# wbhart/mpir-fft

Measured on AMD Instinct MI355X. Metric: limbs/s for new_mpn_mul N×N-bit at 1/2/4/8 MI355X; % HBM roofline, higher is better.
Workload: dtype u64; 1 GPU; C3: new_mpn_mul depth=15 w=4 n1=n2=20312500 limbs (l=2048 limbs/coeff, NC x NR = 256 x 256, trunc=39936); parallelism=single

## Files before the change

### __graft_entry__.py

```python
import os
import subprocess
import sys

ROOT = os.path.dirname(os.path.abspath(__file__))
CSRC = os.path.join(ROOT, "mpir-fft_amd", "csrc")
LIB = os.path.join(ROOT, "mpir-fft_amd", "libmpfft.so")
HIPCC = os.environ.get("HIPCC", "/opt/rocm/bin/hipcc")


def build_lib(force=False):
    if force:
        subprocess.run(["make", "-s", "-C", CSRC, "clean"], check=True)
    jobs = str(min(8, os.cpu_count() or 1))
    subprocess.run(["make", "-s", "-C", CSRC, "-j" + jobs, "HIPCC=" + HIPCC], check=True)
    subprocess.run(["make", "-s", "-C", CSRC, "-j" + jobs, "HIPCC=" + HIPCC, "pwspill"], check=True)


def build_oracle():
    subprocess.run(["make", "-s", "-C", os.path.join(ROOT, "oracle")], check=True)


def build_c_caller():
    subprocess.run(["make", "-s", "-C", os.path.join(ROOT, "tests", "c_abi")], check=True)
    subprocess.run(["make", "-s", "-C", os.path.join(ROOT, "tests", "c_sqr")], check=True)


def build_host_tests():
    subprocess.run(["make", "-s", "-C", os.path.join(ROOT, "tests", "pw_host")], check=True)
    subprocess.run(["make", "-s", "-C", os.path.join(ROOT, "tests", "split_prune_host")], check=True)
    subprocess.run(["make", "-s", "-C", os.path.join(ROOT, "tests", "pw_sqr_host")], check=True)


def build():
    build_lib()
    build_oracle()
    build_c_caller()
    build_host_tests()
    sys.path.insert(0, ROOT)
    import mpfft_loader
    m = mpfft_loader.load()
    assert m.lib().mpfft_version() >= 1


def smoke():
    import numpy as np
    import torch
    sys.path.insert(0, ROOT)
    sys.path.insert(0, os.path.join(ROOT, "oracle"))
    import mpfft_loader
    import oracle as O
    m = mpfft_loader.load()
    assert torch.cuda.is_available(), "smoke() needs a GPU"
    depth, w, n1, n2 = 9, 2, 120, 97
    a = m.fill_random(n1, 0x1001)
    b = m.fill_random(n2, 0x2002)
    dev = torch.device("cuda:0")
    da = torch.from_numpy(a.view(np.int64)).to(dev)
    db = torch.from_numpy(b.view(np.int64)).to(dev)
    dr = torch.zeros(n1 + n2, dtype=torch.int64, device=dev)
    ws = m.alloc_workspace(n1, n2, depth, w, dev)
    m.mul_device(dr, da, n1, db, n2, depth, w, ws)
    torch.cuda.synchronize()
    got = dr.cpu().numpy().view(np.uint64)
    want = O.new_mpn_mul(a, b, depth, w)
    assert (got == want).all(), "GPU new_mpn_mul differs from the oracle"
    assert O.to_int(got) == O.to_int(a) * O.to_int(b), "GPU product is not the exact product"
    r = np.zeros(n1 + n2, dtype=np.uint64)
    m.new_mpn_mul(r, a, n1, b, n2, depth, w)
    assert (r == want).all()
    d6, w6, m1, m2 = 8, 1, 700, 500
    a6 = m.fill_random(m1, 0x61)
    b6 = m.fill_random(m2, 0x62)
    r6 = m.mul6(a6, b6, d6, w6)
    assert (r6 == O.new_mpn_mul6(a6, b6, d6, w6)).all(), "GPU new_mpn_mul6 differs from the oracle"
    assert O.to_int(r6) == O.to_int(a6) * O.to_int(b6)
    ds = torch.zeros(2 * n1, dtype=torch.int64, device=dev)
    wsq = m.alloc_workspace_sqr(n1, depth, w, dev)
    m.sqr_device(ds, da, n1, depth, w, wsq)
    torch.cuda.synchronize()
    assert O.to_int(ds.cpu().numpy().view(np.uint64)) == O.to_int(a) ** 2, "GPU square is not the exact square"
    print("smoke: ok (depth=%d w=%d n1=%d n2=%d; mul6 depth=%d w=%d n1=%d n2=%d)" % (depth, w, n1, n2, d6, w6, m1, m2))


if __name__ == "__main__":
    build()
    if len(sys.argv) > 1 and sys.argv[1] == "smoke":
        smoke()
```

### mpir-fft_amd/csrc/pkernels.hpp

```cpp
#pragma once
#include <type_traits>
#include "coeff.hpp"

#ifndef PW_TIGHT9
#define PW_TIGHT9 1
#endif
__host__ __device__ constexpr bool pw_tight(int K) { return PW_TIGHT9 && K == 512; }
#ifndef PW_LATE_B_ALL
#define PW_LATE_B_ALL 0
#endif
__host__ __device__ constexpr bool pw_late_b(int K) { return pw_tight(K) || PW_LATE_B_ALL; }
#ifndef PW_LATE_INFL
#define PW_LATE_INFL 1
#endif
#ifndef PW_A_INFL
#define PW_A_INFL 2
#endif
#ifndef PW_QUAD4
#define PW_QUAD4 0
#endif

__host__ __device__ constexpr size_t pw_lds_bytes(int M, int K, int l)
{
    return ((size_t)M * K * 8 > (size_t)l * 4 ? (size_t)M * K * 8 : (size_t)l * 4) + (pw_tight(K) ? 0 : (size_t)K * 8);
}

template <int M, int LK>
__host__ __device__ constexpr int pw_wpe()
{
    return pw_lds_bytes(M, 1 << LK, 64 * M) * (1024 >> LK) <= 160 * 1024 ? 4 : 2;
}
#ifndef PW_PD_TIGHT
#define PW_PD_TIGHT 16
#endif
template <int M, int LK>
#ifndef PW_PD_WIDE
#define PW_PD_WIDE 16
#endif
__host__ __device__ constexpr int pw_pd() { return pw_wpe<M, LK>() == 4 ? (pw_tight(1 << LK) ? PW_PD_TIGHT : PW_PD_WIDE) : 2 * M; }


#ifndef PW_NORM_SPILL_ALL
#define PW_NORM_SPILL_ALL 0
#endif
template <int M>
__host__ __device__ __forceinline__ int pw_norm(u64 (&L)[M], int T)
{
    const int D = T + 1;
#if defined(__HIP_DEVICE_COMPILE__)
    {
        const u32 w0 = (u32)L[0], n0 = w0 - (u32)D;
        const bool spill = PW_NORM_SPILL_ALL || (D > 0 ? w0 < (u32)D : (D < 0 ? n0 < (u32)(-D) : false));
        L[0] = (L[0] & ~0xffffffffull) | (spill ? w0 : n0);
        return spill ? T : -1;
    }
#endif
    const u32 dh = D < 0 ? ~0u : 0u;
    u32 b = 0;
#pragma unroll
    for (int j = 0; j < M; ++j) {
        const u32 lo = __builtin_subc((u32)L[j], j == 0 ? (u32)D : dh, b, &b);
        const u32 hi = __builtin_subc((u32)(L[j] >> 32), dh, b, &b);
        L[j] = ((u64)hi << 32) | lo;
    }
    return (D < 0) - (int)b - 1;
}

template <int M, int LK, int PD = 2 * M, int FIXE = -1>
__host__ __device__ __forceinline__ void pw_combine(u64 (&L)[M], int &T, int &S, int alpha, const u32 *Xw,
                                                   int packed, int q, unsigned E)
{
    constexpr int K = 1 << LK, NW = 2 * M;
    constexpr unsigned NP = 64 * M;
    const int Tq = packed >> 1, Sq = packed & 1;
    bool neg = E >= NP;
    if (neg) E -= NP;
    if (FIXE >= 0) E = (unsigned)FIXE;
    const int Yw = ((int)E - 1) >> 5;
    const unsigned sh = (unsigned)(32 * (Yw + 1)) - E;
    if (alpha == 0) {
#pragma unroll
        for (int j = 0; j < M; ++j) L[j] = 0;
        T = 0;
        S = 0;
    } else if (alpha < 0) {
        S ^= 1;
    }
    neg ^= (S ^ Sq) != 0;
    const u32 smask = neg ? ~0u : 0u;
    const u32 *bn = Xw + q - Yw * K;
    const u32 *bw = bn + NW * K;
    u32 wprev = (-1 < Yw ? bw : bn)[-K] ^ (-1 < Yw ? ~smask : smask);
    u32 c = 1;
    constexpr int D0 = PD < NW ? PD : NW;
    u32 wv[NW];
#pragma unroll
    for (int k = 0; k < D0; ++k) {
        const bool wr = k < Yw;
        wv[k] = (wr ? bw : bn)[k * K];
#if defined(__HIP_DEVICE_COMPILE__)
        if ((k & 7) == 7) __builtin_amdgcn_sched_barrier(0);
#endif
    }
#pragma unroll
    for (int k = 0; k < NW; ++k) {
        if (k + D0 < NW) {
            const bool wr2 = k + D0 < Yw;
            wv[k + D0] = (wr2 ? bw : bn)[(k + D0) * K];
        }
        const bool wr = k < Yw;
        const u32 w = wv[k] ^ (wr ? ~smask : smask);
#if defined(__HIP_DEVICE_COMPILE__)
        const u32 o = __builtin_amdgcn_alignbit(w, wprev, sh);
#else
        const u32 o = (u32)((((u64)w << 32) | wprev) >> sh);
#endif
        wprev = w;
        const u32 lw = (u32)(L[k >> 1] >> (32 * (k & 1)));
        const u32 r = __builtin_addc(lw, o, c, &c);
        if (k & 1) L[k >> 1] = (L[k >> 1] & 0xffffffffull) | ((u64)r << 32);
        else L[k >> 1] = (L[k >> 1] & ~0xffffffffull) | r;
#if defined(__HIP_DEVICE_COMPILE__)
        if (D0 < NW && (k & 3) == 3) __builtin_amdgcn_sched_barrier(0);
#endif
    }
    T += (int)c;
    if (Tq != -1) {
        const int cv = neg ? 1 + Tq : -1 - Tq;
        const i64 d = (i64)cv * ((i64)1 << (32 - sh));
        const u32 dl = (u32)d, dhi = (u32)((u64)d >> 32), sx = d < 0 ? ~0u : 0u;
        u32 cc = 0;
#pragma unroll
        for (int k = 0; k < NW; ++k) {
            const u32 ad = k < Yw ? 0u : k == Yw ? dl : k == Yw + 1 ? dhi : sx;
            const u32 lw = (u32)(L[k >> 1] >> (32 * (k & 1)));
            const u32 r = __builtin_addc(lw, ad, cc, &cc);
            if (k & 1) L[k >> 1] = (L[k >> 1] & 0xffffffffull) | ((u64)r << 32);
            else L[k >> 1] = (L[k >> 1] & ~0xffffffffull) | r;
        }
        T += (int)cc + (Yw == NW - 1 ? (int)(d >> 32) : (d < 0 ? -1 : 0));
    }
}

template <int M>
__host__ __device__ __forceinline__ int pw_canon(u64 (&L)[M], int T)
{
    i128 acc = -(i128)T;
#pragma unroll
    for (int j = 0; j < M; ++j) {
        acc += (i128)L[j];
        L[j] = (u64)acc;
        acc >>= 64;
    }
    const int c1 = (int)(i64)acc;
    acc = -(i128)c1;
#pragma unroll
    for (int j = 0; j < M; ++j) {
        acc += (i128)L[j];
        L[j] = (u64)acc;
        acc >>= 64;
    }
    if ((i64)acc != 0) {
#pragma unroll
        for (int j = 0; j < M; ++j) L[j] = 0;
        return 1;
    }
    return 0;
}

template <int M>
__host__ __device__ __forceinline__ void pw_sqrt2(u64 (&L)[M], int &T)
{
    static_assert(M % 2 == 0, "the half swap needs an even limb count");
    constexpr int H = M / 2;
    i128 a0 = (i128)T, a1 = -(i128)T;
#pragma unroll
    for (int j = 0; j < H; ++j) {
        const u64 lo = L[j], hi = L[j + H];
        a0 += -(i128)hi - (i128)lo;
        a1 += (i128)lo - (i128)hi;
        L[j] = (u64)a0;
        L[j + H] = (u64)a1;
        a0 >>= 64;
        a1 >>= 64;
    }
    i128 c = a0;
#pragma unroll
    for (int j = H; j < M; ++j) {
        c += (i128)L[j];
        L[j] = (u64)c;
        c >>= 64;
    }
    T = (int)(i64)(a1 + c);
}

struct PwLdsRef {
    u32 *p;
    int K;
    __device__ __forceinline__ operator u64() const { return ((u64)p[K] << 32) | p[0]; }
    __device__ __forceinline__ PwLdsRef &operator=(u64 v)
    {
        p[0] = (u32)v;
        p[K] = (u32)(v >> 32);
        return *this;
    }
};
struct PwLdsZ {
    u32 *z;
    int K;
    __device__ __forceinline__ PwLdsRef operator[](int j) const { return PwLdsRef{z + 2 * j * K, K}; }
};

template <int M, typename ZT>
__host__ __device__ __forceinline__ void pw_mulmod(ZT &&Z, int &T, const u64 (&La)[M], int ta, const u64 (&Lb)[M], int tb)
{
    if (ta | tb) {
        if (ta && tb) {
#pragma unroll
            for (int j = 0; j < M; ++j) Z[j] = j == 0;
            T = 0;
            return;
        }
        i128 acc = 1;
#pragma unroll
        for (int j = 0; j < M; ++j) {
            acc += (i128)(~(ta ? Lb[j] : La[j]));
            Z[j] = (u64)acc;
            acc >>= 64;
        }
        T = -1 + (int)(i64)acc;
        return;
    }
    constexpr int DB = 29, ND = (64 * M + DB - 1) / DB;
    static_assert(ND < 64, "column sums must stay below 2^64");
    u32 ad[ND], bd[ND];
#pragma unroll
    for (int d = 0; d < ND; ++d) {
        const int b0 = d * DB, li = b0 >> 6, sh = b0 & 63;
        u64 x = La[li] >> sh, y = Lb[li] >> sh;
        if (sh + DB > 64 && li + 1 < M) {
            x |= La[li + 1] << (64 - sh);
            y |= Lb[li + 1] << (64 - sh);
        }
        ad[d] = (u32)(x & ((1u << DB) - 1));
        bd[d] = (u32)(y & ((1u << DB) - 1));
    }
    u128 acc = 0;
    int pos = 0, k = 0;
    i64 bw = 0;
#pragma clang loop unroll(full)
    for (int c = 0; c < 2 * ND - 1; ++c) {
        u64 col = 0;
        const int i0 = c < ND ? 0 : c - ND + 1, i1 = c < ND ? c : ND - 1;
#pragma clang loop unroll(full)
        for (int i = i0; i <= i1; ++i) col += (u64)ad[i] * bd[c - i];
#if defined(__HIP_DEVICE_COMPILE__)
        __builtin_amdgcn_sched_barrier(0);
#endif
        acc += (u128)col << (DB * c - pos);
        const bool last = c == 2 * ND - 2;
#pragma unroll
        for (int e = 0; e < 3; ++e) {
            if (k < 2 * M && (last || DB * (c + 1) - pos >= 64)) {
                const u64 limb = (u64)acc;
                acc >>= 64;
                pos += 64;
                if (k < M) {
                    Z[k] = limb;
                } else {
                    const u64 z = Z[k - M];
                    const u64 d1 = z - limb;
                    i64 b1 = (i64)(d1 > z);
                    const u64 d2 = d1 + (u64)bw;
                    b1 += bw < 0 ? (i64)(d2 > d1) : 0;
                    Z[k - M] = d2;
                    bw = -b1;
                }
                ++k;
            }
        }
    }
    T = (int)bw;
}

template <int M, int LK>
__device__ __forceinline__ void pw_publish_words(const u64 (&L)[M], u32 *Xw, int t)
{
    constexpr int K = 1 << LK;
    u32 *col = Xw + t;
#pragma unroll
    for (int j = 0; j < M; ++j) {
        col[(2 * j) * K] = (u32)L[j];
        col[(2 * j + 1) * K] = (u32)(L[j] >> 32);
    }
}

template <int M, int LK>
__device__ __forceinline__ void pw_publish(u64 (&L)[M], int &T, int S, u32 *Xw, int *TT, int t)
{
    T = pw_norm<M>(L, T);
    pw_publish_words<M, LK>(L, Xw, t);
    if (TT) TT[t] = 2 * T + S;
}

__device__ __forceinline__ unsigned pw_mod(unsigned a, unsigned n)
{
    a = a >= 2 * n ? a - 2 * n : a;
    return a >= n ? a - n : a;
}

__device__ __forceinline__ int pw_launder(int t)
{
#if defined(__HIP_DEVICE_COMPILE__)
    asm volatile("" : "+v"(t));
#endif
    return t;
}

__device__ __forceinline__ void pw_wave_sync()
{
    asm volatile("" ::: "memory");
    __builtin_amdgcn_wave_barrier();
    asm volatile("" ::: "memory");
}

template <int M, int LK, int J, int I = 0>
__device__ __forceinline__ void pw_combine_fixed(u64 (&L)[M], int &T, int &S, int alpha, const u32 *Xw, int packed, int q,
                                                 unsigned E, unsigned Eu)
{
    constexpr unsigned NP = 64 * M;
    constexpr unsigned C = (2 * I + 1) * (NP >> (J + 1));
    if constexpr (I + 1 < (1 << J)) {
        if (Eu == C) {
            pw_combine<M, LK, pw_pd<M, LK>(), (int)C>(L, T, S, alpha, Xw, packed, q, E);
            return;
        }
        pw_combine_fixed<M, LK, J, I + 1>(L, T, S, alpha, Xw, packed, q, E, Eu);
    } else {
        pw_combine<M, LK, pw_pd<M, LK>(), (int)C>(L, T, S, alpha, Xw, packed, q, E);
    }
}

#ifndef PW_UNW_FUSE
#define PW_UNW_FUSE 1
#endif
#ifndef PW_PROBE_NOH1
#define PW_PROBE_NOH1 0
#endif
template <int M, int LK>
__device__ __forceinline__ unsigned pw_unweight_exp(unsigned Pz, unsigned W2, int t)
{
    constexpr unsigned NP = 64 * M, N2 = 2 * NP;
    const bool halff = (W2 & 1) && (t & 1);
    const unsigned un = (((unsigned)t * W2) >> 1) + LK + (halff ? 1 : 0);
    return pw_mod(Pz + N2 - un + (halff ? NP / 4 : 0), N2);
}

template <int M, int LK, int DIR, int FIXJ, bool UNW = false>
__device__ __forceinline__ void pw_level(u64 (&L)[M], int &T, int &S, unsigned &P, u32 *Xw, int *TT, unsigned *PP,
                                         unsigned W2, int t, int jj, bool unw = false)
{
    constexpr int K = 1 << LK, lk = LK;
    constexpr unsigned N2 = 128 * M;
    const int j = DIR == 0 ? jj : lk - 1 - jj;
    const int h = K >> (j + 1);
    const int q = t ^ h;
    const bool top = !(t & h);
    const int qt = t & ~h;
    const unsigned tw = (unsigned)((qt & (h - 1)) << j) * W2;
    const bool cross = h >= 64;
#if PW_PROBE_NOH1
    if (h == 1) {
        u64 cy = P;
#pragma unroll
        for (int m = 0; m < M; ++m) {
            const u64 s = L[m] + cy;
            cy = s < L[m] ? 1 : 0;
            L[m] = s;
        }
        if (!top) P = pw_mod(P + 1, N2);
        return;
    }
#endif
    unsigned Pq;
    int packed;
    if (pw_tight(K)) {
        T = pw_norm<M>(L, T);
        const int own = 2 * T + S;
        if (cross) {
            Xw[t] = (u32)own;
            Xw[K + t] = P;
            __syncthreads();
            packed = (int)Xw[q];
            Pq = Xw[K + q];
            __syncthreads();
        } else {
            packed = __shfl_xor(own, h);
            Pq = (unsigned)__shfl_xor((int)P, h);
        }
        pw_publish_words<M, LK>(L, Xw, t);
        if (cross) __syncthreads(); else pw_wave_sync();
    } else {
        pw_publish<M, LK>(L, T, S, Xw, TT, t);
        PP[t] = P;
        if (cross) __syncthreads(); else pw_wave_sync();
        Pq = PP[q];
        packed = TT[q];
    }
    const int own_packed = 2 * T + S;
    unsigned E;
    if (DIR == 0) {
        E = pw_mod(Pq + N2 - P, N2);
        if constexpr (FIXJ == 0) {
            pw_combine<M, LK, pw_pd<M, LK>(), 32 * M>(L, T, S, top ? 1 : -1, Xw, packed, q, E);
        } else if constexpr (FIXJ > 0) {
            constexpr unsigned NP = 64 * M;
            const unsigned Em = E >= NP ? E - NP : E;
            const unsigned Eu = (unsigned)__builtin_amdgcn_readfirstlane((int)Em);
            pw_combine_fixed<M, LK, FIXJ>(L, T, S, top ? 1 : -1, Xw, packed, q, E, Eu);
        } else {
            pw_combine<M, LK, pw_pd<M, LK>()>(L, T, S, top ? 1 : -1, Xw, packed, q, E);
        }
        if (!top) P = pw_mod(P + tw, N2);
    } else {
        E = top ? pw_mod(Pq + 2 * N2 - tw - P, N2) : pw_mod(Pq + N2 - P + tw, N2);
        if (UNW && unw) {
            if (!top) P = pw_mod(P + N2 - tw, N2);
            const unsigned F = pw_unweight_exp<M, LK>(P, W2, pw_tight(K) ? pw_launder(t) : t);
            constexpr unsigned NP = 64 * M;
            const unsigned Eq = pw_mod(E + F, N2);
            pw_combine<M, LK, pw_pd<M, LK>()>(L, T, S, 0, Xw, own_packed, t, top ? F : pw_mod(F + NP, N2));
            __builtin_amdgcn_sched_barrier(0);
            pw_combine<M, LK, pw_pd<M, LK>()>(L, T, S, 1, Xw, packed, q, Eq);
            P = 0;
        } else {
            pw_combine<M, LK, pw_pd<M, LK>()>(L, T, S, top ? 1 : -1, Xw, packed, q, E);
            if (!top) P = pw_mod(P + N2 - tw, N2);
        }
    }
    if (cross) __syncthreads(); else pw_wave_sync();
}

#ifndef PW_R4_INV
#define PW_R4_INV 0
#endif
template <int M, int LK>
__device__ __forceinline__ void pw_level4_dit(u64 (&L)[M], int &T, int &S, unsigned &P, u32 *Xw, int *TT, unsigned *PP,
                                              unsigned W2, int t, int jj)
{
    constexpr int K = 1 << LK;
    constexpr unsigned NP = 64 * M, N2 = 2 * NP;
    static_assert(!pw_tight(K), "the radix-4 levels use the TT / PP arrays");
    const int jA = LK - 1 - jj, jB = jA - 1;
    const int h1 = K >> (jA + 1), h2 = 2 * h1;
    const int role = ((t & h1) ? 1 : 0) | ((t & h2) ? 2 : 0);
    const int t0 = t & ~(h1 | h2);
    const unsigned A = (unsigned)((t & (h1 - 1)) << jA) * W2;
    const unsigned B = (unsigned)((t & (h2 - 1)) << jB) * W2;
    const bool cross = h2 >= 64;
    pw_publish<M, LK>(L, T, S, Xw, TT, t);
    PP[t] = P;
    if (cross) __syncthreads(); else pw_wave_sync();
    const unsigned eA = A ? N2 - A : 0u, eB = B ? N2 - B : 0u;
    auto ex = [&](int r) -> unsigned { return r == 0 ? 0u : r == 1 ? eA : r == 2 ? eB : pw_mod(eA + eB, N2); };
    const bool n1 = role & 1, n2 = (role >> 1) & 1;
    auto neg = [&](int r) -> bool { return r == 0 ? false : r == 1 ? n1 : r == 2 ? n2 : n1 != n2; };
    const unsigned Pn = pw_mod(P + ex(role), N2);
#pragma unroll
    for (int k = 1; k < 4; ++k) {
        const int r = role ^ k;
        const int q = t0 | ((r & 1) ? h1 : 0) | ((r & 2) ? h2 : 0);
        const unsigned Pq = PP[q];
        const int packed = TT[q];
        unsigned E = pw_mod(Pq + ex(r) + 2 * N2 - Pn, N2);
        if (neg(r)) E = pw_mod(E + NP, N2);
        pw_combine<M, LK, pw_pd<M, LK>()>(L, T, S, k == 1 ? (neg(role) ? -1 : 1) : 1, Xw, packed, q, E);
    }
    P = Pn;
    if (cross) __syncthreads(); else pw_wave_sync();
}

#ifndef PW_R4_FWD
#define PW_R4_FWD 0
#endif
template <int M, int LK>
__device__ __forceinline__ void pw_level4_dif(u64 (&L)[M], int &T, int &S, unsigned &P, u32 *Xw, int *TT, unsigned *PP,
                                              unsigned W2, int t, int jj)
{
    constexpr int K = 1 << LK;
    constexpr unsigned NP = 64 * M, N2 = 2 * NP;
    static_assert(!pw_tight(K), "the radix-4 levels use the TT / PP arrays");
    const int h1 = K >> (jj + 1), h2 = h1 / 2;
    const int role = ((t & h2) ? 1 : 0) | ((t & h1) ? 2 : 0);
    const int t0 = t & ~(h1 | h2);
    const unsigned a0 = (unsigned)((t0 & (h1 - 1)) << jj) * W2, a1 = (unsigned)(((t0 | h2) & (h1 - 1)) << jj) * W2;
    const unsigned B = (unsigned)((t0 & (h2 - 1)) << (jj + 1)) * W2;
    const bool cross = h1 >= 64;
    pw_publish<M, LK>(L, T, S, Xw, TT, t);
    PP[t] = P;
    if (cross) __syncthreads(); else pw_wave_sync();
    auto ex = [&](int i, int r) -> unsigned {
        return pw_mod(((i & 1) ? B : 0u) + ((i & 2) ? ((r & 1) ? a1 : a0) : 0u), N2);
    };
    auto neg = [&](int i, int r) -> bool { return __builtin_popcount(i & r) & 1; };
    const unsigned Pn = pw_mod(P + ex(role, role), N2);
#pragma unroll
    for (int k = 1; k < 4; ++k) {
        const int r = role ^ k;
        const int q = t0 | ((r & 1) ? h2 : 0) | ((r & 2) ? h1 : 0);
        const unsigned Pq = PP[q];
        const int packed = TT[q];
        unsigned E = pw_mod(Pq + ex(role, r) + 2 * N2 - Pn, N2);
        if (neg(role, r)) E = pw_mod(E + NP, N2);
        pw_combine<M, LK, pw_pd<M, LK>()>(L, T, S, k == 1 ? (neg(role, role) ? -1 : 1) : 1, Xw, packed, q, E);
    }
    P = Pn;
    if (cross) __syncthreads(); else pw_wave_sync();
}

#ifndef PW_FIXB
#define PW_FIXB 0
#endif
#ifndef PW_FIXB_EARLY
#define PW_FIXB_EARLY 2
#endif
template <int M, int LK, int DIR, int FIXMAX = 2>
__device__ __forceinline__ void pw_transform(u64 (&L)[M], int &T, int &S, unsigned &P, u32 *Xw, int *TT, unsigned *PP,
                                             unsigned W2, int t)
{
    int jj = 0;
    if (DIR == 0) {
        static_assert(LK >= 7, "level 0's partner K/2 >= 64 lanes away");
        pw_level<M, LK, DIR, 0>(L, T, S, P, Xw, TT, PP, W2, t, 0);
        if constexpr (LK >= 8 && FIXMAX >= 1) pw_level<M, LK, DIR, 1>(L, T, S, P, Xw, TT, PP, W2, t, 1);
        if constexpr (LK >= 9 && FIXMAX >= 2) pw_level<M, LK, DIR, 2>(L, T, S, P, Xw, TT, PP, W2, t, 2);
        jj = LK >= 9 && FIXMAX >= 2 ? 3 : LK >= 8 && FIXMAX >= 1 ? 2 : 1;
    }
    if constexpr (DIR == 1 && PW_R4_INV && !pw_tight(1 << LK)) {
        for (; jj + 1 < LK; jj += 2) pw_level4_dit<M, LK>(L, T, S, P, Xw, TT, PP, W2, t, jj);
    }
    if constexpr (DIR == 0 && PW_R4_FWD && !pw_tight(1 << LK)) {
        for (; jj + 1 < LK; jj += 2) pw_level4_dif<M, LK>(L, T, S, P, Xw, TT, PP, W2, t, jj);
    }
    for (; jj < LK; ++jj) pw_level<M, LK, DIR, -1, DIR == 1 && PW_UNW_FUSE>(L, T, S, P, Xw, TT, PP, W2, t, jj, jj == LK - 1);
}

template <int LP>
struct PwRaw {
    u64 v[LP];
    u64 pw, nw;
    u64 pwp, nwp;
    int top;
};

template <int LP>
__device__ __forceinline__ void pw_piece_fetch(PwRaw<LP> &R, const u64 *dig, const u64 *cbp, const int *topp, int l,
                                               int t)
{
    typedef unsigned long long pw_v2u __attribute__((ext_vector_type(2)));
    static_assert(LP % 2 == 0, "pieces of whole limb pairs");
    const int m0 = t * LP, W = m0 >> 6, mb = m0 ? m0 - 1 : l - 1, Wp = mb >> 6;
#pragma unroll
    for (int j = 0; j < LP; j += 2) {
        const pw_v2u q = *(const pw_v2u *)(dig + m0 + j);
        R.v[j] = q.x;
        R.v[j + 1] = q.y;
    }
    const pw_v2u c = *(const pw_v2u *)(cbp + 2 * W), cp = *(const pw_v2u *)(cbp + 2 * Wp);
    R.pw = c.x;
    R.nw = c.y;
    R.pwp = cp.x;
    R.nwp = cp.y;
    R.top = *topp;
}

template <int M, int LP>
__device__ __forceinline__ void pw_piece_make(u64 (&L)[M], int &T, const PwRaw<LP> &R, int l, int t)
{
    const int m0 = t * LP, b0 = m0 & 63;
    const int mb = m0 ? m0 - 1 : l - 1, bp = mb & 63;
    const int kb = (int)((R.pwp >> bp) & 1) - (int)((R.nwp >> bp) & 1);
    const int cin = m0 ? kb : -kb - R.top;
    i64 c = cin;
#pragma unroll
    for (int j = 0; j < LP; ++j) {
        const u64 v = R.v[j];
        const int k = j ? (int)((R.pw >> (b0 + j - 1)) & 1) - (int)((R.nw >> (b0 + j - 1)) & 1) : 0;
        const i64 add = c + k;
        const u64 r = v + (u64)add;
        c = add >= 0 ? (i64)(r < v) : -(i64)(r > v);
        L[j] = r;
    }
    const u64 up = c < 0 ? ~0ull : 0ull;
#pragma unroll
    for (int j = LP; j < M; ++j) L[j] = j == LP ? (c > 0 ? 1ull : up) : up;
    T = c < 0 ? -1 : 0;
}

template <int M, int LP>
__device__ __forceinline__ void pw_load_piece(u64 (&L)[M], int &T, const u64 *dig, const u64 *cbp, const int *topp,
                                              int l, int t)
{
    PwRaw<LP> R;
    pw_piece_fetch<LP>(R, dig, cbp, topp, l, t);
    pw_piece_make<M, LP>(L, T, R, l, t);
}

template <int M, int LK>
__host__ __device__ constexpr int pw_piece_limbs() { return M <= 12 ? 4 : 8; }

template <int M, int LP>
__device__ __forceinline__ void pw_load_pair_bfly(u64 (&L)[M], int &T, const u64 *dig, const u64 *cb, const int *top,
                                                  long s0, int l, int cbw, int t, bool sub)
{
    u64 A[M], B[M];
    int Ta, Tb;
    {
        PwRaw<LP> RA, RB;
        pw_piece_fetch<LP>(RA, dig + (size_t)s0 * l, cb + (size_t)s0 * cbw, top + s0, l, t);
        pw_piece_fetch<LP>(RB, dig + (size_t)(s0 + 1) * l, cb + (size_t)(s0 + 1) * cbw, top + s0 + 1, l, t);
        pw_piece_make<M, LP>(A, Ta, RA, l, t);
        pw_piece_make<M, LP>(B, Tb, RB, l, t);
    }
    const u32 m = sub ? ~0u : 0u;
    u32 c = sub ? 1u : 0u;
#pragma unroll
    for (int j = 0; j <= LP; ++j) {
        const u32 lo = __builtin_addc((u32)A[j], (u32)B[j] ^ m, c, &c);
        const u32 hi = __builtin_addc((u32)(A[j] >> 32), (u32)(B[j] >> 32) ^ m, c, &c);
        L[j] = ((u64)hi << 32) | lo;
    }
    const u64 up = (i64)L[LP] < 0 ? ~0ull : 0ull;
#pragma unroll
    for (int j = LP + 1; j < M; ++j) L[j] = up;
    T = (i64)L[LP] < 0 ? -1 : 0;
    (void)Ta;
    (void)Tb;
}

template <int M, int LP, int K, int INFL = 2>
__device__ __forceinline__ void pw_load_quad_bfly(u64 (&L)[M], int &T, const u64 *dig, const u64 *cb, const int *top,
                                                  long s0, int pos, int l, int cbw, int t)
{
    u64 acc[LP + 1];
#pragma unroll
    for (int j = 0; j <= LP; ++j) acc[j] = 0;
    const int tr = t ^ (K / 2), sg = t >= K / 2 ? 1 : -1;
    auto sign_of = [&](int q) {
        return q == 0 ? 1 : q == 2 ? (pos < 2 ? 1 : -1)
             : (pos < 2 ? (pos == 0 ? 1 : -1) : (pos == 2 ? sg : -sg) * (q == 1 ? 1 : -1));
    };
    auto add = [&](const PwRaw<LP> &R, int q, int pt) {
        u64 X[M];
        int Tx;
        pw_piece_make<M, LP>(X, Tx, R, l, pt);
        const u32 m = sign_of(q) < 0 ? ~0u : 0u;
        u32 c = m & 1u;
#pragma unroll
        for (int j = 0; j <= LP; ++j) {
            const u32 lo = __builtin_addc((u32)acc[j], (u32)X[j] ^ m, c, &c);
            const u32 hi = __builtin_addc((u32)(acc[j] >> 32), (u32)(X[j] >> 32) ^ m, c, &c);
            acc[j] = ((u64)hi << 32) | lo;
        }
    };
    if (PW_QUAD4 || INFL == 4) {
        const int pr = pos >= 2 ? tr : t;
        PwRaw<LP> R0, R1, R2, R3;
        pw_piece_fetch<LP>(R0, dig + (size_t)s0 * l, cb + (size_t)s0 * cbw, top + s0, l, t);
        pw_piece_fetch<LP>(R2, dig + (size_t)(s0 + 2) * l, cb + (size_t)(s0 + 2) * cbw, top + s0 + 2, l, t);
        pw_piece_fetch<LP>(R1, dig + (size_t)(s0 + 1) * l, cb + (size_t)(s0 + 1) * cbw, top + s0 + 1, l, pr);
        pw_piece_fetch<LP>(R3, dig + (size_t)(s0 + 3) * l, cb + (size_t)(s0 + 3) * cbw, top + s0 + 3, l, pr);
        add(R0, 0, t);
        add(R2, 2, t);
        add(R1, 1, pr);
        add(R3, 3, pr);
    } else if (INFL == 1) {
#pragma unroll
        for (int u = 0; u < 4; ++u) {
            const int q = u < 2 ? 2 * u : 2 * (u - 2) + 1, pt = (q & 1) && pos >= 2 ? tr : t;
            PwRaw<LP> R;
            pw_piece_fetch<LP>(R, dig + (size_t)(s0 + q) * l, cb + (size_t)(s0 + q) * cbw, top + s0 + q, l, pt);
            add(R, q, pt);
        }
    } else
#pragma unroll
    for (int h = 0; h < 2; ++h) {
        const int qa = h, qb = h + 2, pt = h && pos >= 2 ? tr : t;
        PwRaw<LP> Ra, Rb;
        pw_piece_fetch<LP>(Ra, dig + (size_t)(s0 + qa) * l, cb + (size_t)(s0 + qa) * cbw, top + s0 + qa, l, pt);
        pw_piece_fetch<LP>(Rb, dig + (size_t)(s0 + qb) * l, cb + (size_t)(s0 + qb) * cbw, top + s0 + qb, l, pt);
        add(Ra, qa, pt);
        add(Rb, qb, pt);
    }
    const u64 up = (i64)acc[LP] < 0 ? ~0ull : 0ull;
#pragma unroll
    for (int j = 0; j < M; ++j) L[j] = j <= LP ? acc[j] : up;
    T = (i64)acc[LP] < 0 ? -1 : 0;
}

template <int M, int LK, typename LoadB = int>
__device__ __forceinline__ void pw_slot_product(u64 (&La)[M], int Ta, u64 (&Lb)[M], int Tb, u64 *X, u32 *Xw, int *TT,
                                                unsigned *PP, int t, unsigned long long *stamp, LoadB loadB = 0)
{
    constexpr bool late_b = !std::is_same<LoadB, int>::value;
#define PW_STAMP(k) do { if (stamp && t == 0) stamp[k] = __builtin_amdgcn_s_memtime(); } while (0)
    constexpr int K = 1 << LK, lk = LK;
    constexpr unsigned NP = 64 * M, N2 = 2 * NP;
    constexpr unsigned W2 = N2 >> lk;
    static_assert((N2 >> lk) << lk == N2, "omega must be a power of two");
    int Sa = 0, Sb = 0;
    auto weight = [&](int tt) -> unsigned {
        return (((unsigned)tt * W2) >> 1) + (((W2 & 1) && (tt & 1)) ? NP / 4 : 0);
    };
    const bool half = (W2 & 1) && (t & 1);
    unsigned Pa = weight(t), Pb = late_b ? 0u : Pa;
    if (half) {
        pw_sqrt2<M>(La, Ta);
        if (!late_b) pw_sqrt2<M>(Lb, Tb);
    }
    PW_STAMP(1);
    pw_transform<M, LK, 0>(La, Ta, Sa, Pa, Xw, TT, PP, W2, t);
    PW_STAMP(2);
    if constexpr (late_b) {
        loadB(Lb, Tb);
        const int tb = pw_launder(t);
        Pb = weight(tb);
        if ((W2 & 1) && (tb & 1)) pw_sqrt2<M>(Lb, Tb);
    }
    pw_transform<M, LK, 0, late_b ? PW_FIXB : PW_FIXB_EARLY>(Lb, Tb, Sb, Pb, Xw, TT, PP, W2, t);
    PW_STAMP(3);

    const int ca = pw_canon<M>(La, Ta), cb = pw_canon<M>(Lb, Tb);
    u64 Z[M];
    int Tz, Sz = Sa ^ Sb;
    if (pw_tight(K)) {
        pw_mulmod<M>(PwLdsZ{Xw + t, K}, Tz, La, ca, Lb, cb);
#pragma unroll
        for (int j = 0; j < M; ++j) Z[j] = ((u64)Xw[(2 * j + 1) * K + t] << 32) | Xw[2 * j * K + t];
    } else {
        pw_mulmod<M>(Z, Tz, La, ca, Lb, cb);
    }
    unsigned Pz = pw_mod(Pa + Pb, N2);
    PW_STAMP(4);

    pw_transform<M, LK, 1>(Z, Tz, Sz, Pz, Xw, TT, PP, W2, t);
    PW_STAMP(5);
    if constexpr (PW_UNW_FUSE && !(PW_R4_INV && !pw_tight(K) && LK % 2 == 0)) {
        const int tf = pw_tight(K) ? pw_launder(t) : t;
        if ((W2 & 1) && (tf & 1)) pw_sqrt2<M>(Z, Tz);
    } else {
        const int tf = pw_tight(K) ? pw_launder(t) : t;
        const bool halff = (W2 & 1) && (tf & 1);
        const unsigned un = (((unsigned)tf * W2) >> 1) + lk + (halff ? 1 : 0);
        const unsigned F = pw_mod(Pz + N2 - un + (halff ? NP / 4 : 0), N2);
        if (halff) pw_sqrt2<M>(Z, Tz);
        pw_publish<M, LK>(Z, Tz, Sz, Xw, pw_tight(K) ? nullptr : TT, t);
        pw_wave_sync();
        pw_combine<M, LK, pw_pd<M, LK>()>(Z, Tz, Sz, 0, Xw, 2 * Tz + Sz, t, F);
        __syncthreads();
    }
    const int zt = pw_canon<M>(Z, Tz);
    const int neg = zt || (Z[M - 1] >> 63);
    if (pw_tight(K)) {
        u64 b = (u64)neg;
#pragma unroll
        for (int j = 0; j < M; ++j) {
            const u64 z = Z[j];
            X[j * K + t] = z - b;
            b = b && z == 0;
        }
    } else {
#pragma unroll
        for (int j = 0; j < M; ++j) X[j * K + t] = Z[j];
        TT[t] = neg | (zt << 1);
    }
    __syncthreads();
    PW_STAMP(6);
#undef PW_STAMP
}

template <int M, int LK, int NTH = (1 << LK)>
__device__ __forceinline__ void pw_slot_output(const u64 *X, const int *TT, int *H, u64 *pa, u64 *cbp, int *topp, int l,
                                               int t)
{
    constexpr int K = 1 << LK;
    const int LP = l >> LK;
    const int lane = t & 63;
    u64 fo[8];
    int ho[8];
    const int RPT = l / NTH;
#pragma unroll
    for (int r = 0; r < 8; ++r) {
        fo[r] = 0;
        ho[r] = 0;
        if (r >= RPT) continue;
        const int m = t + NTH * r;
        i128 S = 0;
        auto limb_of = [&](int d, int tp) -> i128 {
            i128 v;
            if (pw_tight(K)) {
                v = d < M ? (i128)X[(size_t)d * K + tp] : -(i128)(X[(size_t)(M - 1) * K + tp] >> 63);
            } else {
                const int tt = TT[tp];
                v = d < M ? (i128)X[(size_t)d * K + tp] : (i128)(tt >> 1);
                if ((tt & 1) && (d == 0 || d == M)) v -= 1;
            }
            return v;
        };
        {
            constexpr int LPc = pw_piece_limbs<M, LK>(), KP = M / LPc + 1;
            const int hi = m / LPc;
#pragma unroll
            for (int j = 0; j < KP; ++j) {
                const int tp = hi - j, d = m - tp * LPc;
                if (tp >= 0 && d <= M) S += limb_of(d, tp);
            }
        }
        if (m < M) {
            const int mm = m + l;
            int lo = (mm - M + LP - 1) / LP;
            for (int tp = lo; tp <= K - 1; ++tp) S -= limb_of(mm - tp * LP, tp);
        }
        fo[r] = (u64)S;
        ho[r] = (int)(i64)(S >> 64);
    }
    __syncthreads();
#pragma unroll
    for (int r = 0; r < 8; ++r)
        if (r < RPT) H[t + NTH * r] = ho[r];
    __syncthreads();
#pragma unroll
    for (int r = 0; r < 8; ++r) {
        if (r >= RPT) continue;
        const int m = t + NTH * r;
        const int hin = m ? H[m - 1] : -H[l - 1];
        const u64 f = fo[r];
        const u64 nf = f + (u64)(i64)hin;
        const int kout = hin >= 0 ? (int)(nf < f) : -(int)(nf > f);
        pa[m] = nf;
        const u64 pm = __ballot(kout == 1), nm = __ballot(kout == -1);
        if (lane == 0) {
            cbp[2 * (m >> 6)] = pm;
            cbp[2 * (m >> 6) + 1] = nm;
        }
    }
    if (t == 0) *topp = 0;
}

template <int M, int LK, int FUSE>
__global__ __launch_bounds__(1 << LK) __attribute__((amdgpu_waves_per_eu(pw_wpe<M, LK>()))) void k_pwss(u64 *digA, u64 *cbA, int *topA, const u64 *digB, const u64 *cbB,
                                                  const int *topB, int l, u64 *digC, u64 *cbC, int *topC,
                                                  unsigned long long *dbg)
{
    unsigned long long *stamp = dbg ? dbg + 8 * (size_t)blockIdx.x : nullptr;
    if (stamp && threadIdx.x == 0) stamp[0] = __builtin_amdgcn_s_memtime();
    extern __shared__ __attribute__((aligned(16))) unsigned char smem[];
    constexpr int K = 1 << LK;
    const int t = threadIdx.x;
    u64 *X = (u64 *)smem;
    u32 *Xw = (u32 *)smem;
    int *TT = pw_tight(K) ? nullptr : (int *)(X + (size_t)M * K);
    unsigned *PP = pw_tight(K) ? nullptr : (unsigned *)(TT + K);
    int *H = (int *)smem;
    const int cbw = cb_words(l);
    constexpr int CLP = pw_piece_limbs<M, LK>();
    u64 La[M], Lb[M];
    int Ta = 0, Tb = 0;
    if (FUSE == 0 && pw_late_b(K)) {
        const long slot = blockIdx.x;
        pw_load_piece<M, CLP>(La, Ta, digA + (size_t)slot * l, cbA + (size_t)slot * cbw, topA + slot, l, t);
        auto loadB = [&](u64 (&L)[M], int &T) {
            pw_load_piece<M, CLP>(L, T, digB + (size_t)slot * l, cbB + (size_t)slot * cbw, topB + slot, l, t);
        };
        pw_slot_product<M, LK>(La, Ta, Lb, Tb, X, Xw, TT, PP, t, stamp, loadB);
        pw_slot_output<M, LK>(X, TT, H, digA + (size_t)slot * l, cbA + (size_t)slot * cbw, topA + slot, l, t);
    } else if (FUSE == 0) {
        const long slot = blockIdx.x;
        {
            PwRaw<CLP> RA, RB;
            pw_piece_fetch<CLP>(RA, digA + (size_t)slot * l, cbA + (size_t)slot * cbw, topA + slot, l, t);
            pw_piece_fetch<CLP>(RB, digB + (size_t)slot * l, cbB + (size_t)slot * cbw, topB + slot, l, t);
            pw_piece_make<M, CLP>(La, Ta, RA, l, t);
            pw_piece_make<M, CLP>(Lb, Tb, RB, l, t);
        }
        __syncthreads();
        pw_slot_product<M, LK>(La, Ta, Lb, Tb, X, Xw, TT, PP, t, stamp);
        pw_slot_output<M, LK>(X, TT, H, digA + (size_t)slot * l, cbA + (size_t)slot * cbw, topA + slot, l, t);
    } else if (FUSE == 2) {
        const long b = blockIdx.x, nb = gridDim.x, main = nb - nb % 32;
        long slot = b;
        if (b < main) {
            const long x = b & 7, j = b >> 3;
            slot = 4 * (((j >> 2) << 3) + x) + (j & 3);
        }
        const long s0 = slot & ~3L;
        const int pos = (int)(slot & 3);
        pw_load_quad_bfly<M, CLP, K, PW_A_INFL>(La, Ta, digA, cbA, topA, s0, pos, l, cbw, t);
        if (pw_late_b(K)) {
            auto loadB = [&](u64 (&L)[M], int &T) {
                pw_load_quad_bfly<M, CLP, K, PW_LATE_INFL>(L, T, digB, cbB, topB, s0, pos, l, cbw, pw_launder(t));
            };
            pw_slot_product<M, LK>(La, Ta, Lb, Tb, X, Xw, TT, PP, t, stamp, loadB);
        } else {
            pw_load_quad_bfly<M, CLP, K>(Lb, Tb, digB, cbB, topB, s0, pos, l, cbw, t);
            pw_slot_product<M, LK>(La, Ta, Lb, Tb, X, Xw, TT, PP, t, stamp);
        }
        pw_slot_output<M, LK>(X, TT, H, digC + (size_t)slot * l, cbC + (size_t)slot * cbw, topC + slot, l, t);
    } else {
        const long b = blockIdx.x, nb = gridDim.x, main = nb - nb % 16;
        long slot = b;
        if (b < main) {
            const long x = b & 7, j = b >> 3;
            slot = 2 * (((j >> 1) << 3) + x) + (j & 1);
        }
        pw_load_pair_bfly<M, CLP>(La, Ta, digA, cbA, topA, slot & ~1L, l, cbw, t, slot & 1);
        if (pw_late_b(K)) {
            auto loadB = [&](u64 (&L)[M], int &T) {
                pw_load_pair_bfly<M, CLP>(L, T, digB, cbB, topB, slot & ~1L, l, cbw, t, slot & 1);
            };
            pw_slot_product<M, LK>(La, Ta, Lb, Tb, X, Xw, TT, PP, t, stamp, loadB);
        } else {
            pw_load_pair_bfly<M, CLP>(Lb, Tb, digB, cbB, topB, slot & ~1L, l, cbw, t, slot & 1);
            pw_slot_product<M, LK>(La, Ta, Lb, Tb, X, Xw, TT, PP, t, stamp);
        }
        pw_slot_output<M, LK>(X, TT, H, digC + (size_t)slot * l, cbC + (size_t)slot * cbw, topC + slot, l, t);
    }
    if (stamp) {
        __syncthreads();
        if (threadIdx.x == 0) stamp[7] = __builtin_amdgcn_s_memtime();
    }
}


template <int M, typename ZT>
__host__ __device__ __forceinline__ void pw_sqrmod(ZT &&Z, int &T, const u64 (&La)[M], int ta)
{
    if (ta) {
#pragma unroll
        for (int j = 0; j < M; ++j) Z[j] = j == 0;
        T = 0;
        return;
    }
    constexpr int DB = 29, ND = (64 * M + DB - 1) / DB;
    static_assert(ND < 64, "column sums must stay below 2^64");
    u32 ad[ND];
#pragma unroll
    for (int d = 0; d < ND; ++d) {
        const int b0 = d * DB, li = b0 >> 6, sh = b0 & 63;
        u64 x = La[li] >> sh;
        if (sh + DB > 64 && li + 1 < M) x |= La[li + 1] << (64 - sh);
        ad[d] = (u32)(x & ((1u << DB) - 1));
    }
    u128 acc = 0;
    int pos = 0, k = 0;
    i64 bw = 0;
#pragma clang loop unroll(full)
    for (int c = 0; c < 2 * ND - 1; ++c) {
        u64 off = 0;
        const int i0 = c < ND ? 0 : c - ND + 1;
#pragma clang loop unroll(full)
        for (int i = i0; 2 * i < c; ++i) off += (u64)ad[i] * ad[c - i];
        u64 col = 2 * off;
        if (!(c & 1)) col += (u64)ad[c / 2] * ad[c / 2];
#if defined(__HIP_DEVICE_COMPILE__)
        __builtin_amdgcn_sched_barrier(0);
#endif
        acc += (u128)col << (DB * c - pos);
        const bool last = c == 2 * ND - 2;
#pragma unroll
        for (int e = 0; e < 3; ++e) {
            if (k < 2 * M && (last || DB * (c + 1) - pos >= 64)) {
                const u64 limb = (u64)acc;
                acc >>= 64;
                pos += 64;
                if (k < M) {
                    Z[k] = limb;
                } else {
                    const u64 z = Z[k - M];
                    const u64 d1 = z - limb;
                    i64 b1 = (i64)(d1 > z);
                    const u64 d2 = d1 + (u64)bw;
                    b1 += bw < 0 ? (i64)(d2 > d1) : 0;
                    Z[k - M] = d2;
                    bw = -b1;
                }
                ++k;
            }
        }
    }
    T = (int)bw;
}

template <int M, int LK>
__device__ __forceinline__ void pw_slot_square(u64 (&La)[M], int Ta, u64 *X, u32 *Xw, int *TT, unsigned *PP, int t,
                                               unsigned long long *stamp)
{
#define PW_STAMP(k) do { if (stamp && t == 0) stamp[k] = __builtin_amdgcn_s_memtime(); } while (0)
    constexpr int K = 1 << LK, lk = LK;
    constexpr unsigned NP = 64 * M, N2 = 2 * NP;
    constexpr unsigned W2 = N2 >> lk;
    static_assert((N2 >> lk) << lk == N2, "omega must be a power of two");
    int Sa = 0;
    unsigned Pa = (((unsigned)t * W2) >> 1) + (((W2 & 1) && (t & 1)) ? NP / 4 : 0);
    if ((W2 & 1) && (t & 1)) pw_sqrt2<M>(La, Ta);
    PW_STAMP(1);
    pw_transform<M, LK, 0>(La, Ta, Sa, Pa, Xw, TT, PP, W2, t);
    PW_STAMP(2);
    PW_STAMP(3);

    const int ca = pw_canon<M>(La, Ta);
    u64 Z[M];
    int Tz, Sz = 0;
    if (pw_tight(K)) {
        pw_sqrmod<M>(PwLdsZ{Xw + t, K}, Tz, La, ca);
#pragma unroll
        for (int j = 0; j < M; ++j) Z[j] = ((u64)Xw[(2 * j + 1) * K + t] << 32) | Xw[2 * j * K + t];
    } else {
        pw_sqrmod<M>(Z, Tz, La, ca);
    }
    unsigned Pz = pw_mod(2 * Pa, N2);
    PW_STAMP(4);

    pw_transform<M, LK, 1>(Z, Tz, Sz, Pz, Xw, TT, PP, W2, t);
    PW_STAMP(5);
    if constexpr (PW_UNW_FUSE && !(PW_R4_INV && !pw_tight(K) && LK % 2 == 0)) {
        const int tf = pw_tight(K) ? pw_launder(t) : t;
        if ((W2 & 1) && (tf & 1)) pw_sqrt2<M>(Z, Tz);
    } else {
        const int tf = pw_tight(K) ? pw_launder(t) : t;
        const bool halff = (W2 & 1) && (tf & 1);
        const unsigned un = (((unsigned)tf * W2) >> 1) + lk + (halff ? 1 : 0);
        const unsigned F = pw_mod(Pz + N2 - un + (halff ? NP / 4 : 0), N2);
        if (halff) pw_sqrt2<M>(Z, Tz);
        pw_publish<M, LK>(Z, Tz, Sz, Xw, pw_tight(K) ? nullptr : TT, t);
        pw_wave_sync();
        pw_combine<M, LK, pw_pd<M, LK>()>(Z, Tz, Sz, 0, Xw, 2 * Tz + Sz, t, F);
        __syncthreads();
    }
    const int zt = pw_canon<M>(Z, Tz);
    const int neg = zt || (Z[M - 1] >> 63);
    if (pw_tight(K)) {
        u64 b = (u64)neg;
#pragma unroll
        for (int j = 0; j < M; ++j) {
            const u64 z = Z[j];
            X[j * K + t] = z - b;
            b = b && z == 0;
        }
    } else {
#pragma unroll
        for (int j = 0; j < M; ++j) X[j * K + t] = Z[j];
        TT[t] = neg | (zt << 1);
    }
    __syncthreads();
    PW_STAMP(6);
#undef PW_STAMP
}

template <int M, int LK, int FUSE>
__global__ __launch_bounds__(1 << LK) __attribute__((amdgpu_waves_per_eu(pw_wpe<M, LK>()))) void k_pwsq(u64 *digA, u64 *cbA, int *topA, int l, u64 *digC, u64 *cbC, int *topC,
                                                  unsigned long long *dbg)
{
    unsigned long long *stamp = dbg ? dbg + 8 * (size_t)blockIdx.x : nullptr;
    if (stamp && threadIdx.x == 0) stamp[0] = __builtin_amdgcn_s_memtime();
    extern __shared__ __attribute__((aligned(16))) unsigned char smem[];
    constexpr int K = 1 << LK;
    const int t = threadIdx.x;
    u64 *X = (u64 *)smem;
    u32 *Xw = (u32 *)smem;
    int *TT = pw_tight(K) ? nullptr : (int *)(X + (size_t)M * K);
    unsigned *PP = pw_tight(K) ? nullptr : (unsigned *)(TT + K);
    int *H = (int *)smem;
    const int cbw = cb_words(l);
    constexpr int CLP = pw_piece_limbs<M, LK>();
    u64 La[M];
    int Ta = 0;
    if (FUSE == 0) {
        const long slot = blockIdx.x;
        pw_load_piece<M, CLP>(La, Ta, digA + (size_t)slot * l, cbA + (size_t)slot * cbw, topA + slot, l, t);
        __syncthreads();
        pw_slot_square<M, LK>(La, Ta, X, Xw, TT, PP, t, stamp);
        pw_slot_output<M, LK>(X, TT, H, digA + (size_t)slot * l, cbA + (size_t)slot * cbw, topA + slot, l, t);
    } else if (FUSE == 2) {
        const long b = blockIdx.x, nb = gridDim.x, main = nb - nb % 32;
        long slot = b;
        if (b < main) {
            const long x = b & 7, j = b >> 3;
            slot = 4 * (((j >> 2) << 3) + x) + (j & 3);
        }
        const long s0 = slot & ~3L;
        const int pos = (int)(slot & 3);
        pw_load_quad_bfly<M, CLP, K, PW_A_INFL>(La, Ta, digA, cbA, topA, s0, pos, l, cbw, t);
        pw_slot_square<M, LK>(La, Ta, X, Xw, TT, PP, t, stamp);
        pw_slot_output<M, LK>(X, TT, H, digC + (size_t)slot * l, cbC + (size_t)slot * cbw, topC + slot, l, t);
    } else {
        const long b = blockIdx.x, nb = gridDim.x, main = nb - nb % 16;
        long slot = b;
        if (b < main) {
            const long x = b & 7, j = b >> 3;
            slot = 2 * (((j >> 1) << 3) + x) + (j & 1);
        }
        pw_load_pair_bfly<M, CLP>(La, Ta, digA, cbA, topA, slot & ~1L, l, cbw, t, slot & 1);
        pw_slot_square<M, LK>(La, Ta, X, Xw, TT, PP, t, stamp);
        pw_slot_output<M, LK>(X, TT, H, digC + (size_t)slot * l, cbC + (size_t)slot * cbw, topC + slot, l, t);
    }
    if (stamp) {
        __syncthreads();
        if (threadIdx.x == 0) stamp[7] = __builtin_amdgcn_s_memtime();
    }
}
```

Measured before the change: 5.586 billion limbs/s.

## Use negacyclic Karatsuba for pointwise mulmod/sqrmod at selected limb counts

Replaces the schoolbook 29-bit-digit product modulo 2^N+1 with a one-level Karatsuba scheme for M=18 (and optionally 20 or 10). It computes the low-half, high-half and middle (sum) products and folds them negacyclically, parking the half sums in LDS. The generic path is also rewritten to emit 32-bit words through a shared half-product helper. The goal is fewer 32x32 multiplies per pointwise product, at the cost of extra carry handling, LDS traffic and register pressure.

```diff
diff --git a/__graft_entry__.py b/__graft_entry__.py
--- a/__graft_entry__.py
+++ b/__graft_entry__.py
@@ -29,6 +29,7 @@
     subprocess.run(["make", "-s", "-C", os.path.join(ROOT, "tests", "pw_host")], check=True)
     subprocess.run(["make", "-s", "-C", os.path.join(ROOT, "tests", "split_prune_host")], check=True)
     subprocess.run(["make", "-s", "-C", os.path.join(ROOT, "tests", "pw_sqr_host")], check=True)
+    subprocess.run(["make", "-s", "-C", os.path.join(ROOT, "tests", "pw_mul_host")], check=True)
 
 
 def build():
diff --git a/mpir-fft_amd/csrc/pkernels.hpp b/mpir-fft_amd/csrc/pkernels.hpp
--- a/mpir-fft_amd/csrc/pkernels.hpp
+++ b/mpir-fft_amd/csrc/pkernels.hpp
@@ -211,8 +211,192 @@
     __device__ __forceinline__ PwLdsRef operator[](int j) const { return PwLdsRef{z + 2 * j * K, K}; }
 };
 
-template <int M, typename ZT>
-__host__ __device__ __forceinline__ void pw_mulmod(ZT &&Z, int &T, const u64 (&La)[M], int ta, const u64 (&Lb)[M], int tb)
+template <int M>
+__host__ __device__ __forceinline__ void pw_zword_init(u64 (&Z)[M], int k, u32 w)
+{
+    if (k & 1) Z[k >> 1] |= (u64)w << 32;
+    else Z[k >> 1] = w;
+}
+template <int M>
+__host__ __device__ __forceinline__ void pw_zword_put(u64 (&Z)[M], int k, u32 w)
+{
+    if (k & 1) Z[k >> 1] = (Z[k >> 1] & 0xffffffffull) | ((u64)w << 32);
+    else Z[k >> 1] = (Z[k >> 1] & ~0xffffffffull) | w;
+}
+template <int M>
+__host__ __device__ __forceinline__ u32 pw_zword_get(const u64 (&Z)[M], int k) { return (u32)(Z[k >> 1] >> (32 * (k & 1))); }
+__device__ __forceinline__ void pw_zword_init(const PwLdsZ &Z, int k, u32 w) { Z.z[k * Z.K] = w; }
+__device__ __forceinline__ void pw_zword_put(const PwLdsZ &Z, int k, u32 w) { Z.z[k * Z.K] = w; }
+__device__ __forceinline__ u32 pw_zword_get(const PwLdsZ &Z, int k) { return Z.z[k * Z.K]; }
+
+
+#ifndef PW_KARA_MASK
+#define PW_KARA_MASK 1
+#endif
+template <int M>
+__host__ __device__ constexpr bool pw_kara()
+{
+    return M % 2 == 0 && ((M == 18 && (PW_KARA_MASK & 1)) || (M == 20 && (PW_KARA_MASK & 2)) || (M == 10 && (PW_KARA_MASK & 4)));
+}
+template <int M>
+__host__ __device__ constexpr int pw_kara_db() { return M == 10 ? 30 : 29; }
+
+struct PwParkLds {
+    u32 *z;
+    int K;
+    __device__ __forceinline__ void put(int k, u32 w) { z[k * K] = w; }
+    __device__ __forceinline__ u32 get(int k) const { return z[k * K]; }
+};
+template <int NW>
+struct PwParkReg {
+    u32 w[NW];
+    __host__ __device__ __forceinline__ void put(int k, u32 v) { w[k] = v; }
+    __host__ __device__ __forceinline__ u32 get(int k) const { return w[k]; }
+};
+
+template <int DB, int ND, typename W>
+__host__ __device__ __forceinline__ void pw_digits(u32 (&d)[ND], W word)
+{
+#pragma unroll
+    for (int i = 0; i < ND; ++i) {
+        const int b0 = i * DB, wi = b0 >> 5, sh = b0 & 31;
+        u32 x = word(wi) >> sh;
+        if (sh + DB > 32) x |= word(wi + 1) << (32 - sh);
+        d[i] = x & ((1u << DB) - 1);
+    }
+}
+
+template <int ND, int DB, int NW, bool SQR = false, typename Sink>
+__host__ __device__ __forceinline__ void pw_halfprod(const u32 (&ad)[ND], const u32 (&bd)[ND], Sink &&sink)
+{
+    static_assert(DB < 32 && 3 * DB >= 64 && (unsigned long long)(ND + 1) <= (1ull << (64 - 2 * DB)),
+                  "column sums must stay below 2^64");
+    constexpr int NPC = (32 * NW + DB - 1) / DB;
+    u64 col = 0;
+    u32 cur = 0;
+#pragma clang loop unroll(full)
+    for (int c = 0; c < NPC; ++c) {
+        if (c <= 2 * ND - 2) {
+            const int i0 = c < ND ? 0 : c - ND + 1, i1 = c < ND ? c : ND - 1;
+            if (SQR) {
+#pragma clang loop unroll(full)
+                for (int i = i0; 2 * i < c; ++i) col += (u64)bd[i] * ad[c - i];
+                if (!(c & 1)) col += (u64)ad[c / 2] * ad[c / 2];
+            } else {
+#pragma clang loop unroll(full)
+                for (int i = i0; i <= i1; ++i) col += (u64)ad[i] * bd[c - i];
+            }
+#if defined(__HIP_DEVICE_COMPILE__)
+            __builtin_amdgcn_sched_barrier(0);
+#endif
+        }
+        const u32 dg = (u32)col & ((1u << DB) - 1);
+        col >>= DB;
+        const int bits = (c * DB) & 31, k = (c * DB) >> 5;
+        cur = bits ? cur | (dg << bits) : dg;
+        if (bits + DB >= 32) {
+            if (k < NW) sink(k, cur);
+            cur = dg >> ((32 - bits) & 31);
+        }
+    }
+}
+
+template <int M>
+__host__ __device__ __forceinline__ int pw_kara_fold(u32 (&Zw)[2 * M], int clo, int chi)
+{
+    const int e0 = chi > 0 ? -1 : 0, d = clo + e0;
+    const u32 x0 = e0 ? ~0u : 0u, x1 = d < 0 ? ~0u : 0u;
+    u32 c = 0;
+#pragma unroll
+    for (int k = 0; k < 2 * M; ++k)
+        Zw[k] = __builtin_addc(Zw[k], k == 0 ? (u32)(-chi) : k < M ? x0 : k == M ? (u32)d : x1, c, &c);
+    int top = (int)c - (d < 0 ? 1 : 0);
+    if (top > 0) {
+        u32 b = 1;
+#pragma unroll
+        for (int k = 0; k < 2 * M; ++k) Zw[k] = __builtin_subc(Zw[k], 0u, b, &b);
+        top = -(int)b;
+    }
+    return top;
+}
+
+template <int M, bool SQR, typename ZT, typename PK>
+__host__ __device__ __forceinline__ void pw_kara_product(ZT &&Z, int &T, const u64 (&La)[M], const u64 (&Lb)[M], PK &park)
+{
+    constexpr int DB = pw_kara_db<M>(), ND = (32 * M + 1 + DB - 1) / DB;
+    static_assert(ND == (32 * M + DB - 1) / DB, "the half sums' extra bit must not cost a digit");
+    auto wa = [&](int i) -> u32 { return (u32)(La[i >> 1] >> (32 * (i & 1))); };
+    auto wb = [&](int i) -> u32 { return (u32)(Lb[i >> 1] >> (32 * (i & 1))); };
+    u32 sca = 0, scb = 0;
+#pragma unroll
+    for (int k = 0; k < M; ++k) {
+        park.put(k, __builtin_addc(wa(k), wa(M + k), sca, &sca));
+        if (!SQR) park.put(M + k, __builtin_addc(wb(k), wb(M + k), scb, &scb));
+    }
+    u32 ad[ND], bd[ND];
+    auto second = [&](auto word) {
+        if constexpr (SQR) {
+#pragma unroll
+            for (int i = 0; i < ND; ++i) bd[i] = 2 * ad[i];
+        } else {
+            pw_digits<DB, ND>(bd, word);
+        }
+    };
+    u32 Zw[2 * M];
+    int clo = 0, chi = 0;
+    pw_digits<DB, ND>(ad, [&](int i) -> u32 { return i < M ? wa(i) : 0u; });
+    second([&](int i) -> u32 { return i < M ? wb(i) : 0u; });
+    {
+        u32 c = 0, b = 0;
+        pw_halfprod<ND, DB, 2 * M, SQR>(ad, bd, [&](int k, u32 w) {
+            if (k < M) {
+                Zw[k] = w;
+            } else {
+                const u32 lo = Zw[k - M];
+                Zw[k - M] = __builtin_addc(lo, w, c, &c);
+                Zw[k] = __builtin_subc(w, lo, b, &b);
+            }
+        });
+        clo += (int)c;
+        chi -= (int)b;
+    }
+    pw_digits<DB, ND>(ad, [&](int i) -> u32 { return i < M ? wa(M + i) : 0u; });
+    second([&](int i) -> u32 { return i < M ? wb(M + i) : 0u; });
+    {
+        u32 b1 = 0, b2 = 0, c3 = 0, b4 = 0;
+        pw_halfprod<ND, DB, 2 * M, SQR>(ad, bd, [&](int k, u32 w) {
+            if (k < M) {
+                Zw[k] = __builtin_subc(Zw[k], w, b1, &b1);
+                Zw[M + k] = __builtin_subc(Zw[M + k], w, b2, &b2);
+            } else {
+                Zw[k - M] = __builtin_addc(Zw[k - M], w, c3, &c3);
+                Zw[k] = __builtin_subc(Zw[k], w, b4, &b4);
+            }
+        });
+        clo += (int)c3 - (int)b1;
+        chi -= (int)b2 + (int)b4;
+    }
+    pw_digits<DB, ND>(ad, [&](int i) -> u32 { return i < M ? park.get(i) : i == M ? sca : 0u; });
+    second([&](int i) -> u32 { return i < M ? park.get(M + i) : i == M ? scb : 0u; });
+    {
+        u32 c = 0, b = 0;
+        pw_halfprod<ND, DB, 2 * M + 1, SQR>(ad, bd, [&](int k, u32 w) {
+            if (k < M) Zw[M + k] = __builtin_addc(Zw[M + k], w, c, &c);
+            else if (k < 2 * M) Zw[k - M] = __builtin_subc(Zw[k - M], w, b, &b);
+            else clo -= (int)w;
+        });
+        clo -= (int)b;
+        chi += (int)c;
+    }
+    const int top = pw_kara_fold<M>(Zw, clo, chi);
+#pragma unroll
+    for (int j = 0; j < M; ++j) Z[j] = ((u64)Zw[2 * j + 1] << 32) | Zw[2 * j];
+    T = top;
+}
+
+template <int M, typename ZT, typename PK = PwParkReg<2 * M>>
+__host__ __device__ __forceinline__ void pw_mulmod(ZT &&Z, int &T, const u64 (&La)[M], int ta, const u64 (&Lb)[M], int tb,
+                                                   PK park = PK{})
 {
     if (ta | tb) {
         if (ta && tb) {
@@ -231,56 +415,20 @@
         T = -1 + (int)(i64)acc;
         return;
     }
+    if constexpr (pw_kara<M>()) {
+        pw_kara_product<M, false>(Z, T, La, Lb, park);
+        return;
+    }
     constexpr int DB = 29, ND = (64 * M + DB - 1) / DB;
-    static_assert(ND < 64, "column sums must stay below 2^64");
     u32 ad[ND], bd[ND];
-#pragma unroll
-    for (int d = 0; d < ND; ++d) {
-        const int b0 = d * DB, li = b0 >> 6, sh = b0 & 63;
-        u64 x = La[li] >> sh, y = Lb[li] >> sh;
-        if (sh + DB > 64 && li + 1 < M) {
-            x |= La[li + 1] << (64 - sh);
-            y |= Lb[li + 1] << (64 - sh);
-        }
-        ad[d] = (u32)(x & ((1u << DB) - 1));
-        bd[d] = (u32)(y & ((1u << DB) - 1));
-    }
-    u128 acc = 0;
-    int pos = 0, k = 0;
-    i64 bw = 0;
-#pragma clang loop unroll(full)
-    for (int c = 0; c < 2 * ND - 1; ++c) {
-        u64 col = 0;
-        const int i0 = c < ND ? 0 : c - ND + 1, i1 = c < ND ? c : ND - 1;
-#pragma clang loop unroll(full)
-        for (int i = i0; i <= i1; ++i) col += (u64)ad[i] * bd[c - i];
-#if defined(__HIP_DEVICE_COMPILE__)
-        __builtin_amdgcn_sched_barrier(0);
-#endif
-        acc += (u128)col << (DB * c - pos);
-        const bool last = c == 2 * ND - 2;
-#pragma unroll
-        for (int e = 0; e < 3; ++e) {
-            if (k < 2 * M && (last || DB * (c + 1) - pos >= 64)) {
-                const u64 limb = (u64)acc;
-                acc >>= 64;
-                pos += 64;
-                if (k < M) {
-                    Z[k] = limb;
-                } else {
-                    const u64 z = Z[k - M];
-                    const u64 d1 = z - limb;
-                    i64 b1 = (i64)(d1 > z);
-                    const u64 d2 = d1 + (u64)bw;
-                    b1 += bw < 0 ? (i64)(d2 > d1) : 0;
-                    Z[k - M] = d2;
-                    bw = -b1;
-                }
-                ++k;
-            }
-        }
-    }
-    T = (int)bw;
+    pw_digits<DB, ND>(ad, [&](int i) -> u32 { return i < 2 * M ? (u32)(La[i >> 1] >> (32 * (i & 1))) : 0u; });
+    pw_digits<DB, ND>(bd, [&](int i) -> u32 { return i < 2 * M ? (u32)(Lb[i >> 1] >> (32 * (i & 1))) : 0u; });
+    u32 bw = 0;
+    pw_halfprod<ND, DB, 4 * M>(ad, bd, [&](int k, u32 w) {
+        if (k < 2 * M) pw_zword_init(Z, k, w);
+        else pw_zword_put(Z, k - 2 * M, __builtin_subc(pw_zword_get(Z, k - 2 * M), w, bw, &bw));
+    });
+    T = -(int)bw;
 }
 
 template <int M, int LK>
@@ -733,7 +881,9 @@
     const int ca = pw_canon<M>(La, Ta), cb = pw_canon<M>(Lb, Tb);
     u64 Z[M];
     int Tz, Sz = Sa ^ Sb;
-    if (pw_tight(K)) {
+    if constexpr (pw_kara<M>()) {
+        pw_mulmod<M>(Z, Tz, La, ca, Lb, cb, PwParkLds{Xw + t, K});
+    } else if (pw_tight(K)) {
         pw_mulmod<M>(PwLdsZ{Xw + t, K}, Tz, La, ca, Lb, cb);
 #pragma unroll
         for (int j = 0; j < M; ++j) Z[j] = ((u64)Xw[(2 * j + 1) * K + t] << 32) | Xw[2 * j * K + t];
@@ -932,13 +1082,17 @@
 }
 
 
-template <int M, typename ZT>
-__host__ __device__ __forceinline__ void pw_sqrmod(ZT &&Z, int &T, const u64 (&La)[M], int ta)
+template <int M, typename ZT, typename PK = PwParkReg<2 * M>>
+__host__ __device__ __forceinline__ void pw_sqrmod(ZT &&Z, int &T, const u64 (&La)[M], int ta, PK park = PK{})
 {
     if (ta) {
 #pragma unroll
         for (int j = 0; j < M; ++j) Z[j] = j == 0;
         T = 0;
+        return;
+    }
+    if constexpr (pw_kara<M>()) {
+        pw_kara_product<M, true>(Z, T, La, La, park);
         return;
     }
     constexpr int DB = 29, ND = (64 * M + DB - 1) / DB;
@@ -1011,7 +1165,9 @@
     const int ca = pw_canon<M>(La, Ta);
     u64 Z[M];
     int Tz, Sz = 0;
-    if (pw_tight(K)) {
+    if constexpr (pw_kara<M>()) {
+        pw_sqrmod<M>(Z, Tz, La, ca, PwParkLds{Xw + t, K});
+    } else if (pw_tight(K)) {
         pw_sqrmod<M>(PwLdsZ{Xw + t, K}, Tz, La, ca);
 #pragma unroll
         for (int j = 0; j < M; ++j) Z[j] = ((u64)Xw[(2 * j + 1) * K + t] << 32) | Xw[2 * j * K + t];
```

Measured after the change: 5.652 billion limbs/s (median of 6 runs). +1.2%, better.
